# meyer-lab/cmtf-pls

Measured on AMD Instinct MI355X. Metric: nipals_iters_per_sec, higher is better.
Workload: dtype f32

## Files before the change

### cmtf_pls_amd/_lib.py

```python
from __future__ import annotations

import ctypes
import os
from ctypes import c_char_p, c_double, c_int, c_int64, c_size_t, c_uint64, c_void_p

_HERE = os.path.dirname(os.path.abspath(__file__))
LIB_PATH = os.environ.get("CMTFPLS_LIB") or os.path.join(_HERE, "lib", "libcmtfpls.so")

_P = c_void_p

class XcovBlock(ctypes.Structure):
    _fields_ = [("S", _P), ("S2", _P), ("colcnt", _P), ("n_samples", c_double), ("order", c_int), ("A", c_int), ("B", c_int),
                ("n_squarings", c_int), ("Z", _P), ("wA", _P), ("wB", _P), ("info", _P)]


class KfoldState(ctypes.Structure):
    _fields_ = [("I", c_int), ("A", c_int), ("B", c_int), ("M", c_int), ("K", c_int), ("R", c_int)] + [
        (name, _P) for name in ("fold_of", "S", "mean", "Yk", "Gy", "WA", "WB", "Q", "Wa", "Wb", "T", "Gt", "coef", "Rm", "tm",
                                "Tout", "vec", "n_iter", "status", "part")]


SIGNATURES = {
    "cmtfpls_xcov_iterate_blocks_f64": (c_int, [ctypes.POINTER(XcovBlock), c_int, c_int, _P, _P, _P, _P, _P, c_int, _P, c_size_t, _P]),
    "cmtfpls_abi_version": (c_int, []),
# ... 33 lines not shown
    "cmtfpls_project_rows2_f32": (c_int, [_P, c_int, c_int, _P, _P, _P, _P, c_int, c_int, _P, _P, _P, c_int64, c_int, _P, c_int, _P]),
    "cmtfpls_project_rows2_f64": (c_int, [_P, c_int, c_int, _P, _P, _P, _P, c_int, c_int, _P, _P, _P, c_int64, c_int, _P, c_int, _P]),
    "cmtfpls_project_rows_idx_f32": (c_int, [_P, _P, c_int64, c_int, c_int, c_int, _P, _P, _P, _P, c_int, _P]),
    "cmtfpls_project_rows_idx_f64": (c_int, [_P, _P, c_int64, c_int, c_int, c_int, _P, _P, _P, _P, c_int, _P]),
    "cmtfpls_project_rows2_idx_f32": (c_int, [_P, c_int, c_int, _P, _P, _P, _P, c_int, c_int, _P, _P, _P, _P, c_int64, c_int, _P, c_int, _P]),
    "cmtfpls_project_rows2_idx_f64": (c_int, [_P, c_int, c_int, _P, _P, _P, _P, c_int, c_int, _P, _P, _P, _P, c_int64, c_int, _P, c_int, _P]),
    "cmtfpls_allreduce_sum_f64": (c_int, [_P, _P, c_size_t, _P]),
    "cmtfpls_allreduce_sum_f32": (c_int, [_P, _P, c_size_t, _P]),
    "cmtfpls_axpy_scalar_f64": (c_int, [_P, c_int64, _P, _P, _P]),
    "cmtfpls_xcov_deflate_f32": (c_int, [_P, c_int64, c_int, c_int, _P, c_int, c_int, _P, _P, _P, _P, _P, _P, c_size_t, _P]),
    "cmtfpls_xcov_deflate_f64": (c_int, [_P, c_int64, c_int, c_int, _P, c_int, c_int, _P, _P, _P, _P, _P, _P, c_size_t, _P]),
    "cmtfpls_xcov_stats_workspace_bytes": (c_size_t, [c_int64, c_int64, c_int]),
    "cmtfpls_xcov_stats_f32": (c_int, [_P, c_int64, c_int64, _P, c_int, c_int, _P, _P, _P, c_size_t, _P]),
    "cmtfpls_xcov_stats_f64": (c_int, [_P, c_int64, c_int64, _P, c_int, c_int, _P, _P, _P, c_size_t, _P]),
    "cmtfpls_xcov_ssq_workspace_bytes": (c_size_t, [c_int64, c_int64, c_int]),
    "cmtfpls_xcov_ssq_f32": (c_int, [_P, c_int64, c_int64, _P, c_int, c_int, _P, _P, _P, _P, c_size_t, _P]),
    "cmtfpls_xcov_ssq_f64": (c_int, [_P, c_int64, c_int64, _P, c_int, c_int, _P, _P, _P, _P, c_size_t, _P]),
    "cmtfpls_score_contract_workspace_bytes": (c_size_t, [c_int64, c_int64]),
    "cmtfpls_score_contract_f32": (c_int, [_P, c_int64, c_int, c_int, _P, _P, _P, _P, _P, c_double, _P, _P, _P, _P, c_size_t, _P]),
    "cmtfpls_score_contract_f64": (c_int, [_P, c_int64, c_int, c_int, _P, _P, _P, _P, _P, c_double, _P, _P, _P, _P, c_size_t, _P]),
    "cmtfpls_kr_axpy_f64": (c_int, [_P, c_int, c_int, _P, _P, c_int, c_int, _P, _P]),
    "cmtfpls_xcov_f32_mixed": (c_int, [_P, c_int64, c_int64, _P, c_int, c_int, _P, c_int, _P, c_size_t, _P]),
    "cmtfpls_mttkrp_f32_mixed": (c_int, [_P, c_int64, c_int, c_int, _P, _P, c_int, _P, c_int, _P]),
    "cmtfpls_mttkrp_f32": (c_int, [_P, c_int64, c_int, c_int, _P, _P, c_int, _P, c_int, _P]),
    "cmtfpls_mttkrp_f64": (c_int, [_P, c_int64, c_int, c_int, _P, _P, c_int, _P, c_int, _P]),
    "cmtfpls_score_f32": (c_int, [_P, c_int64, c_int, c_int, _P, _P, _P, _P, _P]),
    "cmtfpls_score_f64": (c_int, [_P, c_int64, c_int, c_int, _P, _P, _P, _P, _P]),
    "cmtfpls_score_s_f64": (c_int, [_P, c_int, c_int, c_int, _P, _P, _P, _P]),
    "cmtfpls_deflate_contract_workspace_bytes": (c_size_t, [c_int64, c_int64]),
    "cmtfpls_deflate_contract_yq_f32": (c_int, [_P, c_int64, c_int, c_int, _P, _P, _P, _P, c_int, c_int, _P, _P, c_int, _P, _P, c_size_t, _P]),
    "cmtfpls_deflate_contract_yq_f64": (c_int, [_P, c_int64, c_int, c_int, _P, _P, _P, _P, c_int, c_int, _P, _P, c_int, _P, _P, c_size_t, _P]),
    "cmtfpls_score_gram_f32": (c_int, [_P, c_int64, c_int, c_int, _P, _P, _P, _P, _P, c_int, c_int, _P, _P]),
    "cmtfpls_score_gram_f64": (c_int, [_P, c_int64, c_int, c_int, _P, _P, _P, _P, _P, c_int, c_int, _P, _P]),
    "cmtfpls_q_update_f64": (c_int, [_P, c_int, c_int, _P, c_int, _P, _P, _P, _P]),
    "cmtfpls_deflate_f32": (c_int, [_P, c_int64, c_int, c_int, _P, _P, _P, _P, _P]),
    "cmtfpls_deflate_f64": (c_int, [_P, c_int64, c_int, c_int, _P, _P, _P, _P, _P]),
    "cmtfpls_score_deflate_f32": (c_int, [_P, c_int64, c_int, c_int, _P, _P, _P, _P, _P, _P]),
    "cmtfpls_score_deflate_f64": (c_int, [_P, c_int64, c_int, c_int, _P, _P, _P, _P, _P, _P]),
    "cmtfpls_small_workspace_bytes": (c_size_t, []),
    "cmtfpls_gram_tn_f64": (c_int, [_P, c_int, c_int, _P, c_int, c_int, c_int64, _P, _P, c_size_t, _P]),
    "cmtfpls_rowdot_f64": (c_int, [_P, c_int, c_int, c_int64, _P, _P, _P, _P, _P, c_size_t, _P]),
    "cmtfpls_scores_mean_f64": (c_int, [_P, c_int, c_int64, _P, _P]),
    "cmtfpls_y_deflate_f64": (c_int, [_P, c_int, c_int, c_int64, _P, c_int, c_int, _P, _P, _P, _P, c_size_t, _P]),
    "cmtfpls_sum_f64": (c_int, [_P, c_int64, _P, _P]),
    "cmtfpls_normal_solve_f64": (c_int, [_P, _P, c_int, _P, c_int, _P]),
    "cmtfpls_normal_solve_workspace_bytes": (c_size_t, [c_int]),
    "cmtfpls_normal_solve_ws_f64": (c_int, [_P, _P, c_int, _P, c_int, _P, c_size_t, _P]),
    "cmtfpls_unit_upper_solve_rows_f64": (c_int, [_P, c_int64, c_int, c_int, _P, _P, _P, _P]),
    "cmtfpls_kr_gram_row_f64": (c_int, [_P, c_int, c_int, c_int, _P, c_int, _P]),
    "cmtfpls_kr_gram_f64": (c_int, [_P, c_int, c_int, _P, c_int, c_double, _P]),
    "cmtfpls_khatri_rao_f64": (c_int, [_P, c_int, _P, c_int, c_int, _P, _P]),
    "cmtfpls_predict_rows_f64": (c_int, [_P, c_int64, c_int, c_int, _P, c_int, _P, _P, c_int, _P]),
    "cmtfpls_recon_f32": (c_int, [_P, c_int64, c_int, c_int, _P, _P, c_int, c_int, _P, _P, _P]),
    "cmtfpls_recon_f64": (c_int, [_P, c_int64, c_int, c_int, _P, _P, c_int, c_int, _P, _P, _P]),
    "cmtfpls_recon_r2_workspace_bytes": (c_size_t, [c_int64, c_int64]),
    "cmtfpls_recon_r2_f32": (c_int, [_P, _P, c_int64, c_int, c_int, _P, _P, c_int, c_int, _P, _P, _P, c_size_t, _P]),
    "cmtfpls_recon_r2_f64": (c_int, [_P, _P, c_int64, c_int, c_int, _P, _P, c_int, c_int, _P, _P, _P, c_size_t, _P]),
    "cmtfpls_resid_rows_workspace_bytes": (c_size_t, [c_int64, c_int64]),
    "cmtfpls_resid_rows_f32": (c_int, [_P, _P, c_int64, c_int, c_int, _P, _P, c_int, c_int, _P, _P, _P, _P, c_size_t, _P]),
    "cmtfpls_resid_rows_f64": (c_int, [_P, _P, c_int64, c_int, c_int, _P, _P, c_int, c_int, _P, _P, _P, _P, c_size_t, _P]),
    "cmtfpls_loo_fold_workspace_bytes": (c_size_t, [c_int, c_int, c_int, c_int, c_int]),
    "cmtfpls_loo_tpls_f64": (c_int, [_P, _P, _P, _P, c_int, c_int, c_int, c_int, c_int, c_double, c_int, c_int, c_int, _P, _P, _P, c_size_t, _P]),
    "cmtfpls_loo_xcov_fold_workspace_bytes": (c_size_t, [c_int, c_int, c_int, c_int, c_int]),
    "cmtfpls_kfold_xcov_workspace_bytes": (c_size_t, [c_int64, c_int64, c_int, c_int]),
    "cmtfpls_kfold_xcov_f32": (c_int, [_P, c_int64, c_int, c_int, _P, c_int, _P, _P, c_int, _P, _P, _P, _P, _P, c_size_t, _P]),
    "cmtfpls_kfold_xcov_f64": (c_int, [_P, c_int64, c_int, c_int, _P, c_int, _P, _P, c_int, _P, _P, _P, _P, _P, c_size_t, _P]),
# ... 59 lines not shown
```

### cmtf_pls_amd/backend.py

```python
from __future__ import annotations

import ctypes
from typing import Optional, Tuple

import torch

from . import _lib

_SUFFIX = {torch.float32: "f32", torch.float64: "f64"}


def _ptr(t: Optional[torch.Tensor]):
    return None if t is None else t.data_ptr()


class HipBackend:
    name = "hip"

    def __init__(self, device: Optional[torch.device] = None):
        self.lib = _lib.load()
        if not torch.cuda.is_available():
            raise _lib.CmtfplsError("cmtf_pls_amd needs a ROCm GPU (torch.cuda.is_available() is False); there is no CPU fallback")
        self.device = torch.device(device) if device is not None else torch.device("cuda", torch.cuda.current_device())
        self.n_partials = int(self.lib.cmtfpls_sweep_partials())
# ... 274 lines not shown
        assert WA.is_contiguous() and WB.is_contiguous() and out.stride(1) == 1
        fn = self.lib.cmtfpls_mttkrp_f32_mixed if (mixed and X2.dtype == torch.float32) else self._fn("mttkrp", X2)
        rc = fn(_ptr(X2), X2.shape[0], A, B, _ptr(WA), _ptr(WB), R, _ptr(out), out.stride(0), self._stream())
        if rc == 4:
            return None
        _lib.check(rc, "mttkrp")
        return out

    def score(self, X2, A, B, wA, wB, rowcnt, out) -> torch.Tensor:
        _lib.check(self._fn("score", X2)(_ptr(X2), X2.shape[0], A, B, _ptr(wA), _ptr(wB), _ptr(rowcnt), _ptr(out), self._stream()), "score")
        return out

    def score_s(self, S, A, B, wA, wB, out) -> torch.Tensor:
        assert S.dtype == torch.float64 and S.is_contiguous()
        _lib.check(self.lib.cmtfpls_score_s_f64(_ptr(S), S.shape[0], A, B, _ptr(wA), _ptr(wB), _ptr(out), self._stream()), "score_s")
        return out

    def score_contract(self, X2, A, B, wA, wB, shift, t, Z, sub_own=None, add_other=None, alpha: float = 1.0,
                       csum: Optional[torch.Tensor] = None) -> Optional[torch.Tensor]:
        I, P = X2.shape
        if not X2.is_contiguous() or P != A * B:
            return None
        for v in (sub_own, add_other):
            assert v is None or (v.is_contiguous() and v.numel() == I and v.dtype == torch.float64)
        nbytes = self.lib.cmtfpls_score_contract_workspace_bytes(I, P)
        ws = self._workspace("score_contract", max(nbytes, 256))
        rc = self._fn("score_contract", X2)(_ptr(X2), I, A, B, _ptr(wA), _ptr(wB), _ptr(shift), _ptr(sub_own), _ptr(add_other), float(alpha),
                                            _ptr(t), _ptr(Z), _ptr(csum), _ptr(ws), ws.numel(), self._stream())
        if rc == 4:
            return None
        _lib.check(rc, "score_contract")
        return Z

    def score_gram(self, X2, A, B, wA, wB, rowcnt, out, Y: torch.Tensor, qpart: torch.Tensor) -> Optional[torch.Tensor]:
        assert qpart.numel() >= self.n_partials * Y.shape[1] and qpart.is_contiguous()
        rc = self._fn("score_gram", X2)(_ptr(X2), X2.shape[0], A, B, _ptr(wA), _ptr(wB), _ptr(rowcnt), _ptr(out),
                                        _ptr(Y), Y.stride(0), Y.shape[1], _ptr(qpart), self._stream())
        if rc == 4:
            return None
        _lib.check(rc, "score_gram")
        return out

    def q_update(self, q: torch.Tensor, qpart: Optional[torch.Tensor] = None, normalize: bool = True,
                 G: Optional[torch.Tensor] = None, q_prev: Optional[torch.Tensor] = None,
                 du2: Optional[torch.Tensor] = None, nparts: Optional[int] = None) -> None:
        M = q.numel()
        nrows = (nparts or self.n_partials) if qpart is not None else 0
        assert qpart is None or (qpart.is_contiguous() and qpart.numel() >= nrows * M)
        _lib.check(self.lib.cmtfpls_q_update_f64(_ptr(qpart), nrows, M, _ptr(q), int(normalize),
                                                 _ptr(G), _ptr(q_prev), _ptr(du2), self._stream()), "q_update")

    def deflate(self, X2, A, B, t, wA, wB) -> torch.Tensor:
        part = self.empty(self.n_partials)
        _lib.check(self._fn("deflate", X2)(_ptr(X2), X2.shape[0], A, B, _ptr(t), _ptr(wA), _ptr(wB), _ptr(part), self._stream()), "deflate")
        return self._close_partials(part)

    def deflate_contract_yq(self, X2, A, B, t, wA, wB, Y: torch.Tensor, q: torch.Tensor, masked: bool,
                            out: torch.Tensor) -> Optional[torch.Tensor]:
        I, P = X2.shape
        ws = self._workspace("deflate_contract", self.lib.cmtfpls_deflate_contract_workspace_bytes(I, P))
        ssq = self.empty(1)
        rc = self._fn("deflate_contract_yq", X2)(_ptr(X2), I, A, B, _ptr(t), _ptr(wA), _ptr(wB), _ptr(Y), Y.stride(0), Y.shape[1],
                                                 _ptr(q), _ptr(out), int(masked), _ptr(ssq), _ptr(ws), ws.numel(), self._stream())
        if rc == 4:
            return None
        _lib.check(rc, "deflate_contract_yq")
        return ssq

    def score_deflate(self, X2, A, B, wA, wB, rowcnt, out) -> Optional[torch.Tensor]:
        part = self.empty(self.n_partials)
# ... 351 lines not shown
```

### cmtf_pls_amd/csrc/sweeps.hip

```cpp
#include "common.hpp"

namespace cmtfpls {

#ifndef CMTFPLS_CONTRACT_U
#define CMTFPLS_CONTRACT_U 4
#endif
constexpr int kContractU = CMTFPLS_CONTRACT_U;
constexpr int kYqChunk = 2048;
#ifndef CMTFPLS_YQ_UNFUSE_TILES
#define CMTFPLS_YQ_UNFUSE_TILES 16
#endif
constexpr int kYqUnfuseTiles = CMTFPLS_YQ_UNFUSE_TILES;

struct ContractPlan {
  int vec;
  int col_tiles;
  int row_blocks;
  int rows_per_block;
};

constexpr int kDcU = 2;

#ifndef CMTFPLS_CONTRACT_BLOCKS_FULL
#define CMTFPLS_CONTRACT_BLOCKS_FULL 512
// ... 610 lines not shown
      hipLaunchKernelGGL((deflate_contract_kernel<T, 0, false>), grid, dim3(kSweepThreads), 0, st, X, I, P, B, t, wA, wB, u_ws,
                         part, sspart, p.rows_per_block, nullptr, 0, 0, nullptr);
  } else if (masked)
    hipLaunchKernelGGL((deflate_contract_kernel<T, 1, true>), grid, dim3(kSweepThreads), lds, st, X, I, P, B, t, wA, wB, nullptr,
                       part, sspart, p.rows_per_block, Y, ldy, M, q);
  else
    hipLaunchKernelGGL((deflate_contract_kernel<T, 0, true>), grid, dim3(kSweepThreads), lds, st, X, I, P, B, t, wA, wB, nullptr,
                       part, sspart, p.rows_per_block, Y, ldy, M, q);
  launch_reduce_rows(part, p.row_blocks, P, Z, st);
  launch_reduce_rows(sspart, (int)nss, 1, ssq, st);
  return check_launch("deflate_contract_yq");
}

__device__ __forceinline__ void stage_loadings(double* sA, double* sB, const double* __restrict__ wA,
                                               const double* __restrict__ wB, int A, int B) {
  for (int i = threadIdx.x; i < A; i += blockDim.x) sA[i] = wA[i];
  for (int i = threadIdx.x; i < B; i += blockDim.x) sB[i] = wB[i];
  __syncthreads();
}
static inline size_t loadings_lds_bytes(int A, int B) { return ((size_t)((A + 1) & ~1) + (size_t)((B + 1) & ~1)) * sizeof(double); }

template <typename T, int V, bool MASKED>
__device__ __forceinline__ double dot_pack(const Pack<T, V>& x, const double* sBk) {
  double s = 0.0;
#pragma unroll
  for (int e = 0; e < V; ++e) {
    T xv = x.e[e];
    if (MASKED) xv = (xv == xv) ? xv : (T)0;
    s = fma((double)xv, sBk[e], s);
  }
  return s;
}

template <typename T, bool MASKED, bool VEC, bool GRAM, bool GL = false>
__global__ __launch_bounds__(kSweepThreads) __attribute__((amdgpu_waves_per_eu(5))) void score_kernel(
    const T* __restrict__ X, int64_t I, int A, int B, const double* __restrict__ wA,
    const double* __restrict__ wB, const double* __restrict__ rowcnt, double* __restrict__ t,
    const double* __restrict__ Y, int ldy, int M, double* __restrict__ qpart) {
  extern __shared__ double lds[];
  __shared__ double qs[kSweepThreads / kWave][kWave];
  double qacc = 0.0;
  const double* sA = GL ? wA : lds;
  const double* sB = GL ? wB : lds + ((A + 1) & ~1);
  if (!GL) stage_loadings(lds, lds + ((A + 1) & ~1), wA, wB, A, B);
  constexpr int V = VEC ? VecOf<T>::N : 1;
  using VT = Pack<T, V>;
  const int lane = threadIdx.x & 63;
  const int64_t P = (int64_t)A * B;
  const int64_t nwaves = (int64_t)gridDim.x * (kSweepThreads / kWave);
  const int64_t step = (int64_t)kWave * V;
  const int64_t c0 = (int64_t)lane * V;
  const KronWalk w0(c0, step, B);
  for (int64_t row = (int64_t)blockIdx.x * (kSweepThreads / kWave) + (threadIdx.x >> 6); row < I; row += nwaves) {
    const T* __restrict__ xr = X + row * P;
    double yv = 0.0;
    if (GRAM) yv = Y[row * ldy + ((lane < M) ? lane : 0)];
    double acc = 0.0;
    KronWalk w = w0;
    int64_t c = c0;
    constexpr int UN = kRowUnroll;
    for (; c + (UN - 1) * step < P; c += UN * step) {
      VT x[UN];
#pragma unroll
      for (int s = 0; s < UN; ++s) x[s] = ld_stream(reinterpret_cast<const VT*>(xr + c + s * step));
#pragma unroll
      for (int s = 0; s < UN; ++s) {
        acc = fma(sA[w.j], dot_pack<T, V, MASKED>(x[s], sB + w.k), acc);
        w.next();
      }
    }
    for (; c < P; c += step) {
      const VT x = ld_stream(reinterpret_cast<const VT*>(xr + c));
      acc = fma(sA[w.j], dot_pack<T, V, MASKED>(x, sB + w.k), acc);
      w.next();
    }
    acc = wave_sum(acc);
    const double ti = MASKED ? acc / rowcnt[row] * (double)P : acc;
    if (lane == 0) t[row] = ti;
    if (GRAM) qacc = fma(ti, yv, qacc);
  }
  if (GRAM) {
    qs[threadIdx.x >> 6][lane] = qacc;
    __syncthreads();
    if (threadIdx.x < M) {
      double tot = 0.0;
#pragma unroll
      for (int wv = 0; wv < kSweepThreads / kWave; ++wv) tot += qs[wv][threadIdx.x];
      qpart[(int64_t)blockIdx.x * M + threadIdx.x] = tot;
    }
  }
}

template <typename T, bool MASKED>
__global__ __launch_bounds__(1024) void score_fewrows_kernel(const T* __restrict__ X, int A, int B, const double* __restrict__ wA,
                                                            const double* __restrict__ wB, const double* __restrict__ rowcnt,
                                                            double* __restrict__ t) {
  extern __shared__ double lds[];
  __shared__ double red[16];
  const double* sA = lds;
  const double* sB = lds + ((A + 1) & ~1);
  stage_loadings(lds, lds + ((A + 1) & ~1), wA, wB, A, B);
  constexpr int V = VecOf<T>::N;
  using VT = Pack<T, V>;
  const int64_t P = (int64_t)A * B;
  const int64_t step = (int64_t)1024 * V;
  const int64_t row = blockIdx.x;
  const T* __restrict__ xr = X + row * P;
  KronWalk w((int64_t)threadIdx.x * V, step, B);
  double acc = 0.0;
  int64_t c = (int64_t)threadIdx.x * V;
  constexpr int UN = 4;
  for (; c + (UN - 1) * step < P; c += UN * step) {
    VT x[UN];
#pragma unroll
    for (int s = 0; s < UN; ++s) x[s] = ld_stream(reinterpret_cast<const VT*>(xr + c + s * step));
#pragma unroll
    for (int s = 0; s < UN; ++s) {
      acc = fma(sA[w.j], dot_pack<T, V, MASKED>(x[s], sB + w.k), acc);
      w.next();
    }
  }
// ... 367 lines not shown
template <typename T>
static int narrow_nvl(const T* X, int A, int B) {
#ifndef CMTFPLS_ROWS_NARROW
#define CMTFPLS_ROWS_NARROW 1
#endif
  constexpr int V = VecOf<T>::N;
  if (!CMTFPLS_ROWS_NARROW || (B % V) != 0 || (reinterpret_cast<uintptr_t>(X) & 15) != 0) return 0;
  const int64_t P = (int64_t)A * B;
  if (P <= 64 * V) return 1;
  if (P <= 2 * 64 * V) return 2;
  if (P <= 4 * 64 * V) return 4;
  return 0;
}

template <typename T, bool MASKED, bool GRAM, int OP>
static void launch_rows_narrow(int nvl, hipStream_t st, T* X, int64_t I, int A, int B, const double* wA, const double* wB,
                               const double* rowcnt, double* t, const double* Y, int ldy, int M, double* qpart, double* ssq_part) {
  const dim3 g(kSweepBlocks), b(kSweepThreads);
  if (nvl == 1) hipLaunchKernelGGL((rows_narrow_kernel<T, MASKED, GRAM, 1, OP>), g, b, 0, st, X, I, A, B, wA, wB, rowcnt, t, Y, ldy, M, qpart, ssq_part);
  else if (nvl == 2) hipLaunchKernelGGL((rows_narrow_kernel<T, MASKED, GRAM, 2, OP>), g, b, 0, st, X, I, A, B, wA, wB, rowcnt, t, Y, ldy, M, qpart, ssq_part);
  else hipLaunchKernelGGL((rows_narrow_kernel<T, MASKED, GRAM, 4, OP>), g, b, 0, st, X, I, A, B, wA, wB, rowcnt, t, Y, ldy, M, qpart, ssq_part);
}

template <typename T>
static bool vec_ok(const T* X, int B) {
  return (B % VecOf<T>::N == 0) && ((reinterpret_cast<uintptr_t>(X) & 15) == 0);
}
static bool shape_ok(int64_t I, int A, int B) { return I > 0 && A > 0 && B > 0; }
static constexpr size_t kMaxLoadingsLds = 96 * 1024;

template <typename T>
static int run_score(const T* X, int64_t I, int A, int B, const double* wA, const double* wB,
                     const double* rowcnt, double* t, hipStream_t st,
                     const double* Y = nullptr, int ldy = 0, int M = 0, double* qpart = nullptr, bool few_rows_ok = false) {
  if (!X || !wA || !wB || !t || !shape_ok(I, A, B)) { set_error("score: bad argument"); return CMTFPLS_EINVAL; }
  const bool gram = Y != nullptr;
  if (gram && (!qpart || M <= 0 || ldy < M)) { set_error("score_gram: bad argument"); return CMTFPLS_EINVAL; }
  if (gram && M > kWave) { set_error("score_gram: more than 64 responses; use score + gram_tn"); return CMTFPLS_EUNSUPPORTED; }
  if (const int nvl = narrow_nvl(X, A, B)) {
    T* Xm = const_cast<T*>(X);
    const bool msk = rowcnt != nullptr;
    if (gram) { if (msk) launch_rows_narrow<T, true, true, 0>(nvl, st, Xm, I, A, B, wA, wB, rowcnt, t, Y, ldy, M, qpart, nullptr);
                else launch_rows_narrow<T, false, true, 0>(nvl, st, Xm, I, A, B, wA, wB, rowcnt, t, Y, ldy, M, qpart, nullptr); }
    else      { if (msk) launch_rows_narrow<T, true, false, 0>(nvl, st, Xm, I, A, B, wA, wB, rowcnt, t, nullptr, 0, 0, nullptr, nullptr);
                else launch_rows_narrow<T, false, false, 0>(nvl, st, Xm, I, A, B, wA, wB, rowcnt, t, nullptr, 0, 0, nullptr, nullptr); }
    return check_launch("score");
  }
  size_t lds = loadings_lds_bytes(A, B);
  const bool gl = lds > kMaxLoadingsLds;
  if (gl) lds = 0;
  const bool v = vec_ok(X, B), m = rowcnt != nullptr;
  if (few_rows_ok && !gram && v && !gl && I <= 64 && (int64_t)A * B >= 8192) {
    if (m) hipLaunchKernelGGL((score_fewrows_kernel<T, true>), dim3((unsigned)I), dim3(1024), lds, st, X, A, B, wA, wB, rowcnt, t);
    else hipLaunchKernelGGL((score_fewrows_kernel<T, false>), dim3((unsigned)I), dim3(1024), lds, st, X, A, B, wA, wB, rowcnt, t);
    return check_launch("score");
  }
  const dim3 g(kSweepBlocks), b(kSweepThreads);
#define LAUNCH(MS, V, G) do { if (gl) hipLaunchKernelGGL((score_kernel<T, MS, V, G, true>), g, b, lds, st, X, I, A, B, wA, wB, rowcnt, t, Y, ldy, M, qpart); \
    else hipLaunchKernelGGL((score_kernel<T, MS, V, G, false>), g, b, lds, st, X, I, A, B, wA, wB, rowcnt, t, Y, ldy, M, qpart); } while (0)
  if (gram) { if (m && v) LAUNCH(true, true, true); else if (m) LAUNCH(true, false, true); else if (v) LAUNCH(false, true, true); else LAUNCH(false, false, true); }
  else      { if (m && v) LAUNCH(true, true, false); else if (m) LAUNCH(true, false, false); else if (v) LAUNCH(false, true, false); else LAUNCH(false, false, false); }
#undef LAUNCH
  return check_launch("score");
}

template <typename T>
static int run_deflate(T* X, int64_t I, int A, int B, const double* t, const double* wA, const double* wB,
                       double* ssq_part, hipStream_t st) {
  if (!X || !wA || !wB || !t || !shape_ok(I, A, B)) { set_error("deflate: bad argument"); return CMTFPLS_EINVAL; }
  if (const int nvl = narrow_nvl(X, A, B)) {
    launch_rows_narrow<T, false, false, 1>(nvl, st, X, I, A, B, wA, wB, nullptr, const_cast<double*>(t), nullptr, 0, 0, nullptr, ssq_part);
    return check_launch("deflate");
  }
  const size_t lds = loadings_lds_bytes(A, B);
  const dim3 g(kSweepBlocks), b(kSweepThreads);
  if (lds > kMaxLoadingsLds) {
    if (vec_ok(X, B)) hipLaunchKernelGGL((deflate_kernel<T, true, true>), g, b, 0, st, X, I, A, B, t, wA, wB, ssq_part);
    else hipLaunchKernelGGL((deflate_kernel<T, false, true>), g, b, 0, st, X, I, A, B, t, wA, wB, ssq_part);
    return check_launch("deflate");
  }
#ifndef CMTFPLS_DEFLATE_ROWS
#define CMTFPLS_DEFLATE_ROWS 1
#endif
  if (CMTFPLS_DEFLATE_ROWS && vec_ok(X, B)) {
    const int64_t P = (int64_t)A * B;
    constexpr int V = VecOf<T>::N;
    const bool kc = ((1024 * V) % B) == 0;
#ifndef CMTFPLS_DEFLATE_ROWS_PAD
#define CMTFPLS_DEFLATE_ROWS_PAD 81920
#endif
    const size_t lds_w = loadings_lds_bytes(A, B);
    const size_t lds = lds_w + ((lds_w + CMTFPLS_DEFLATE_ROWS_PAD + 1024 <= 160 * 1024) ? CMTFPLS_DEFLATE_ROWS_PAD : 0);
    if (P > (int64_t)256 * V * 4 && P <= (int64_t)1024 * V * 4) {
      if (kc) hipLaunchKernelGGL((deflate_rows_kernel<T, 4, 1024, true>), g, dim3(1024), lds, st, X, I, A, B, t, wA, wB, ssq_part);
// ... 120 lines not shown
    else launch_rows_narrow<T, false, false, 2>(nvl, st, X, I, A, B, wA, wB, rowcnt, t, nullptr, 0, 0, nullptr, ssq_part);
    return check_launch("score_deflate");
  }
  const size_t lds = loadings_lds_bytes(A, B);
  if (lds > kMaxLoadingsLds) { set_error("score_deflate: loadings exceed LDS"); return CMTFPLS_EUNSUPPORTED; }
  const bool v = vec_ok(X, B), m = rowcnt != nullptr;
  const int V = v ? VecOf<T>::N : 1;
  const int64_t P = (int64_t)A * B;
  int threads = 256, nv = 1;
  if (P > (int64_t)256 * V * 4) { threads = 1024; nv = 4; }
  if (P > (int64_t)1024 * V * 16) { set_error("score_deflate: row does not fit one workgroup; use score + deflate"); return CMTFPLS_EUNSUPPORTED; }
  while ((int64_t)threads * V * nv < P) nv *= 4;
  if (threads == 1024 && nv == 16 && lds + (size_t)1024 * 8 * 16 + 1024 > (size_t)160 * 1024) {
    set_error("score_deflate: loadings + the parked half row exceed the LDS; use score + deflate");
    return CMTFPLS_EUNSUPPORTED;
  }
  const bool kc = v && ((threads * V) % B == 0);
  const bool full = kc && ((int64_t)threads * V * nv == P);
  if (m && full) launch_sd<T, true, true, 2>(nv, threads, lds, st, X, I, A, B, wA, wB, rowcnt, t, ssq_part);
  else if (m && kc) launch_sd<T, true, true, 1>(nv, threads, lds, st, X, I, A, B, wA, wB, rowcnt, t, ssq_part);
  else if (m && v) launch_sd<T, true, true, 0>(nv, threads, lds, st, X, I, A, B, wA, wB, rowcnt, t, ssq_part);
  else if (m) launch_sd<T, true, false, 0>(nv, threads, lds, st, X, I, A, B, wA, wB, rowcnt, t, ssq_part);
  else if (full) launch_sd<T, false, true, 2>(nv, threads, lds, st, X, I, A, B, wA, wB, rowcnt, t, ssq_part);
  else if (kc) launch_sd<T, false, true, 1>(nv, threads, lds, st, X, I, A, B, wA, wB, rowcnt, t, ssq_part);
  else if (v) launch_sd<T, false, true, 0>(nv, threads, lds, st, X, I, A, B, wA, wB, rowcnt, t, ssq_part);
  else launch_sd<T, false, false, 0>(nv, threads, lds, st, X, I, A, B, wA, wB, rowcnt, t, ssq_part);
  return check_launch("score_deflate");
}

}

using namespace cmtfpls;

extern "C" {

int cmtfpls_sweep_partials(void) { return kSweepBlocks; }

size_t cmtfpls_mode0_contract_workspace_bytes(int64_t I, int64_t P) {
  if (I <= 0 || P <= 0) return 0;
  int rb = 1;
  for (int elem = 4; elem <= 8; elem += 4)
    for (int U = 2; U <= kContractU; U += 2)
      for (int which = 0; which < 2; ++which) {
        const int r = plan_contract(I, P, elem, U, which ? kContractBlocks : kContractBlocksFull).row_blocks;
        if (r > rb) rb = r;
      }
  return (size_t)rb * (size_t)P * sizeof(double) + (size_t)I * sizeof(double);
}
size_t cmtfpls_colstats_workspace_bytes(int64_t I, int64_t P) { return 2 * cmtfpls_mode0_contract_workspace_bytes(I, P); }

int cmtfpls_colstats_f32(const float* X, int64_t I, int64_t P, double* colsum, double* colcnt, void* ws, size_t n, void* s) {
  return run_contract<float, 2>(X, I, P, nullptr, colsum, colcnt, ws, n, (hipStream_t)s);
}
int cmtfpls_colstats_f64(const double* X, int64_t I, int64_t P, double* colsum, double* colcnt, void* ws, size_t n, void* s) {
  return run_contract<double, 2>(X, I, P, nullptr, colsum, colcnt, ws, n, (hipStream_t)s);
}
int cmtfpls_mode0_contract_f32(const float* X, int64_t I, int64_t P, const double* u, double* Z, int masked, void* ws, size_t n, void* s) {
  return masked ? run_contract<float, 1>(X, I, P, u, Z, nullptr, ws, n, (hipStream_t)s)
                : run_contract<float, 0>(X, I, P, u, Z, nullptr, ws, n, (hipStream_t)s);
}
int cmtfpls_mode0_contract_f64(const double* X, int64_t I, int64_t P, const double* u, double* Z, int masked, void* ws, size_t n, void* s) {
  return masked ? run_contract<double, 1>(X, I, P, u, Z, nullptr, ws, n, (hipStream_t)s)
                : run_contract<double, 0>(X, I, P, u, Z, nullptr, ws, n, (hipStream_t)s);
}
int cmtfpls_mode0_contract_yq_f32(const float* X, int64_t I, int64_t P, const double* Y, int ldy, int M, const double* q,
                                  double* Z, int masked, void* ws, size_t n, void* s) {
// ... 3 lines not shown
int cmtfpls_mode0_contract_yq_f64(const double* X, int64_t I, int64_t P, const double* Y, int ldy, int M, const double* q,
                                  double* Z, int masked, void* ws, size_t n, void* s) {
  return masked ? run_contract<double, 1>(X, I, P, nullptr, Z, nullptr, ws, n, (hipStream_t)s, Y, ldy, M, q)
                : run_contract<double, 0>(X, I, P, nullptr, Z, nullptr, ws, n, (hipStream_t)s, Y, ldy, M, q);
}
size_t cmtfpls_deflate_contract_workspace_bytes(int64_t I, int64_t P) {
  if (I <= 0 || P <= 0) return 0;
  const ContractPlan a = plan_contract(I, P, 4, kDcU), b = plan_contract(I, P, 8, kDcU);
  const size_t na = (size_t)a.row_blocks * ((size_t)P + a.col_tiles), nb = (size_t)b.row_blocks * ((size_t)P + b.col_tiles);
  const size_t colform = ((na > nb ? na : nb) + (size_t)I) * sizeof(double);
  const size_t rowform = ((size_t)kDcRowsGrid * (size_t)P + (size_t)kDcRowsGrid + (size_t)I) * sizeof(double);
  return colform > rowform ? colform : rowform;
}
int cmtfpls_deflate_contract_yq_f32(float* X, int64_t I, int A, int B, const double* t, const double* wA, const double* wB,
                                    const double* Y, int ldy, int M, const double* q, double* Z, int masked, double* ssq,
                                    void* ws, size_t n, void* s) {
  return run_deflate_contract<float>(X, I, A, B, t, wA, wB, Y, ldy, M, q, Z, masked, ssq, ws, n, (hipStream_t)s);
}
int cmtfpls_deflate_contract_yq_f64(double* X, int64_t I, int A, int B, const double* t, const double* wA, const double* wB,
                                    const double* Y, int ldy, int M, const double* q, double* Z, int masked, double* ssq,
                                    void* ws, size_t n, void* s) {
  return run_deflate_contract<double>(X, I, A, B, t, wA, wB, Y, ldy, M, q, Z, masked, ssq, ws, n, (hipStream_t)s);
}
int cmtfpls_score_gram_f32(const float* X, int64_t I, int A, int B, const double* wA, const double* wB, const double* rowcnt,
                           double* t, const double* Y, int ldy, int M, double* qpart, void* s) {
  if (!Y) { set_error("score_gram: Y is null"); return CMTFPLS_EINVAL; }
  return run_score<float>(X, I, A, B, wA, wB, rowcnt, t, (hipStream_t)s, Y, ldy, M, qpart);
}
int cmtfpls_score_gram_f64(const double* X, int64_t I, int A, int B, const double* wA, const double* wB, const double* rowcnt,
                           double* t, const double* Y, int ldy, int M, double* qpart, void* s) {
  if (!Y) { set_error("score_gram: Y is null"); return CMTFPLS_EINVAL; }
  return run_score<double>(X, I, A, B, wA, wB, rowcnt, t, (hipStream_t)s, Y, ldy, M, qpart);
}
int cmtfpls_center_f32(float* X, int64_t I, int64_t P, const double* mean, double* rowcnt, double* ssq_part, void* s) {
  return run_center<float>(X, I, P, mean, rowcnt, ssq_part, (hipStream_t)s);
}
int cmtfpls_center_f64(double* X, int64_t I, int64_t P, const double* mean, double* rowcnt, double* ssq_part, void* s) {
  return run_center<double>(X, I, P, mean, rowcnt, ssq_part, (hipStream_t)s);
}
int cmtfpls_score_f32(const float* X, int64_t I, int A, int B, const double* wA, const double* wB, const double* rowcnt, double* t, void* s) {
  return run_score<float>(X, I, A, B, wA, wB, rowcnt, t, (hipStream_t)s);
}
int cmtfpls_score_s_f64(const double* S, int M, int A, int B, const double* wA, const double* wB, double* tq, void* s) {
  return run_score<double>(S, M, A, B, wA, wB, nullptr, tq, (hipStream_t)s, nullptr, 0, 0, nullptr, true);
}
int cmtfpls_score_f64(const double* X, int64_t I, int A, int B, const double* wA, const double* wB, const double* rowcnt, double* t, void* s) {
  return run_score<double>(X, I, A, B, wA, wB, rowcnt, t, (hipStream_t)s);
}
int cmtfpls_deflate_f32(float* X, int64_t I, int A, int B, const double* t, const double* wA, const double* wB, double* ssq_part, void* s) {
  return run_deflate<float>(X, I, A, B, t, wA, wB, ssq_part, (hipStream_t)s);
}
int cmtfpls_deflate_f64(double* X, int64_t I, int A, int B, const double* t, const double* wA, const double* wB, double* ssq_part, void* s) {
  return run_deflate<double>(X, I, A, B, t, wA, wB, ssq_part, (hipStream_t)s);
}
int cmtfpls_score_deflate_f32(float* X, int64_t I, int A, int B, const double* wA, const double* wB, const double* rowcnt, double* t, double* ssq_part, void* s) {
  return run_score_deflate<float>(X, I, A, B, wA, wB, rowcnt, t, ssq_part, (hipStream_t)s);
}
int cmtfpls_score_deflate_f64(double* X, int64_t I, int A, int B, const double* wA, const double* wB, const double* rowcnt, double* t, double* ssq_part, void* s) {
  return run_score_deflate<double>(X, I, A, B, wA, wB, rowcnt, t, ssq_part, (hipStream_t)s);
}

}
```

### cmtf_pls_amd/fitrun.py

```python
from __future__ import annotations

import math
from typing import Dict, List, Optional

import numpy as np
import torch

from .fitrun_xcov import XcovMixin
from .state import BlockState, FitState, split_trailing, validate_limits


class FitRun(XcovMixin):

    def __init__(self, eng: NipalsEngine, Xs: List[torch.Tensor], Y: torch.Tensor, n_components: int, coupled: bool,
                 algorithm: str = "direct", owned: Optional[List[bool]] = None, allow_raw: bool = True):
        be, comm = eng.be, eng.comm
        Xs = list(Xs)
        owned = [True] * len(Xs) if owned is None else list(owned)
        if algorithm not in ("direct", "xcov"):
            raise ValueError("algorithm must be 'direct' or 'xcov'")
        self.algorithm_requested = self.algorithm = algorithm
        self.notes: List[str] = []
        validate_limits([tuple(X.shape) for X in Xs], n_components)
        self.eng, self.Xs, self.Y, self.R, self.coupled = eng, Xs, Y, n_components, coupled
# ... 66 lines not shown
        self.Zs = [be.empty(blk.A * blk.B) for blk in self.blocks]
        self.fac = [be.zeros(len(blk.shape) - 1, max(blk.shape[1:])) if len(blk.shape) > 3 else None for blk in self.blocks]
        self.tol = 1e-8
        self.Ts = be.empty(len(self.blocks), I)
        self.t = self.Ts[0] if (len(self.blocks) == 1 and not coupled) else be.empty(I)
        self.status = be.zeros(1 + 2 * len(self.blocks))
        self.status[1::2] = 1.0
        self.status_host = None
        if self.status.is_cuda:
            self.status_host = torch.empty(self.status.shape, dtype=torch.float64, pin_memory=True)
        self.sq_max = int(getattr(be, "rank1_squarings", 30))
        self.sq_budget = [self.sq_max] * len(self.blocks)
        side = int(getattr(be, "rank1_chain_side", 0))
        self.sq_spare = [3 if (len(blk.shape) == 3 and min(blk.A, blk.B) <= side) else 1 for blk in self.blocks]
        self.u = be.empty(I)
        self.u_new = be.empty(I)
        self.q = be.empty(M)
        self.n_iter: List[int] = []
        self.pipeline_stats = {"iterations": 0, "ahead": 0, "unused": 0, "waited": 0, "redone": 0}
        self._executed = 0
        self._parity = 0
        self.mixed = False
        self.use_graphs = False
        self._graphs = {}
        self._graph_error = None
        self._collectives_captured = None
        self._z_ready = False
        self._fused = (algorithm == "direct" and M <= 64
                       and all(hasattr(be, f) for f in ("mode0_contract_yq", "score_gram", "q_update")))
        if self._fused:
            self.Gy = be.empty(M, M)
            self.qbuf = [be.zeros(M), be.zeros(M)]
            self.qpart = be.empty(len(self.blocks), int(be.n_partials) * M)
        elif algorithm == "direct" and comm.sharded:
            self.Gy = be.empty(M, M)
            self.q_prev = be.zeros(M)
        if algorithm == "xcov":
            nb = len(self.blocks)
            self._s_pair = 2 * M <= 64 and eng.opt.xcov_pair_build
            self.S, self.S2, self.S12 = [], [], []
            for blk in self.blocks:
                if blk.has_miss and self._s_pair:
                    both = be.empty(2 * M, blk.A * blk.B)
                    self.S12.append(both)
                    self.S.append(both[:M])
                    self.S2.append(both[M:])
                else:
                    self.S12.append(None)
                    pre = self._s_prebuilt.get(len(self.S))
                    self.S.append(pre if pre is not None else be.empty(M, blk.A * blk.B))
                    self.S2.append(be.empty(M, blk.A * blk.B) if blk.has_miss else None)
            self.rowscale = [(float(blk.A * blk.B) / blk.rowcnt) if blk.has_miss else None for blk in self.blocks]
            any_miss = any(blk.has_miss for blk in self.blocks)
            self.Yw = be.empty(I, 2 * M if self._s_pair else M) if any_miss else None
            self.Gy = be.empty(M, M)
            self.Tq = be.empty(nb, M)
            self.qx = [be.zeros(M), be.zeros(M)]
            self.qc = self.qx[0]
            self.qn = self.Tq[0] if (nb == 1 and not coupled) else be.empty(M)
            self._s_carry = (not any(blk.has_miss for blk in self.blocks)
                             and all(hasattr(be, f) for f in ("s_downdate", "deflate_contract_yq")))
            self._s_ready = False
            self._nowrite = False
            if self.raw:
                self.zM = be.zeros(M)
                self.zA = [be.zeros(blk.A) for blk in self.blocks]
# ... 252 lines not shown
                    seg_colscale()
                self._run(("loadings", budgets), seg_loadings_scores)
                comm.allreduce(self.q)
                self._run(("yupdate", it > 0, par), seg_y_update)
            host = self._read_status()
            local, peer = self._update_budgets(host), self._peer_failed(host, first)
            if not (local or peer):
                break
            first = False
        if sharded:
            self.q_prev.copy_(self.q)
        self._parity ^= 1
        return None if it == 0 else math.sqrt(max(float(host[0]), 0.0))

    def _iterate_fused(self, it: int) -> Optional[float]:
        be, comm = self.eng.be, self.eng.comm
        self._executed += 1
        sharded = comm.sharded
        par = self._parity
        q_cur, q_new = self.qbuf[par], self.qbuf[par ^ 1]
        nparts = len(self.blocks) * int(be.n_partials)

        def seg_contract():
            for b, blk in enumerate(self.blocks):
                if be.mode0_contract_yq(self.X2[b], self.Y, q_cur, blk.has_miss, out=self.Zs[b]) is None:
                    be.rowdot(self.Y, q_cur, self.u, None)
                    be.mode0_contract(self.X2[b], self.u, blk.has_miss, out=self.Zs[b])

        def seg_colscale():
            for b, blk in enumerate(self.blocks):
                if blk.has_miss:
                    be.colscale(self.Zs[b], blk.colcnt, self.n_total)

        def seg_loadings_scores():
            for b, blk in enumerate(self.blocks):
                self.eng._rank1(blk, self.Zs[b], self.wA[b], self.wB[b], info=self.status[1 + 2 * b: 3 + 2 * b],
                                n_squarings=self.sq_budget[b], fac=self.fac[b], tol=self.tol)
                if be.score_gram(self.X2[b], blk.A, blk.B, self.wA[b], self.wB[b], blk.rowcnt if blk.has_miss else None,
                                 self.Ts[b], self.Y, self.qpart[b]) is None:
                    raise RuntimeError("score_gram refused a shape the fused iteration was planned for")
            if sharded:
                be.q_update(q_new, self.qpart, normalize=False, nparts=nparts)

        def seg_y_update():
            if sharded:
                be.q_update(q_new, None, normalize=True, G=self.Gy, q_prev=q_cur, du2=self.status[0:1])
            else:
                be.q_update(q_new, self.qpart, normalize=True, G=self.Gy, q_prev=q_cur, du2=self.status[0:1], nparts=nparts)

        have_z = self._z_ready and it == 0
        self._z_ready = False
        first = True
        while True:
            budgets = tuple(self.sq_budget)
            if not sharded:
                def whole():
                    if first:
                        if not have_z:
                            seg_contract()
                        seg_colscale()
                    seg_loadings_scores()
                    seg_y_update()
                self._run(("fiter", par, budgets, first, have_z), whole)
            else:
                def whole_sharded():
                    if first:
                        if not have_z:
                            seg_contract()
                        for b in range(len(self.blocks)):
                            comm.allreduce(self.Zs[b])
                        seg_colscale()
                    seg_loadings_scores()
                    comm.allreduce(q_new)
                    seg_y_update()
                if not self._run_with_collectives(("fiter+ar", par, budgets, first, have_z), whole_sharded):
                    if first:
                        if not have_z:
                            self._run(("fcontract", par), seg_contract)
                        for b in range(len(self.blocks)):
                            comm.allreduce(self.Zs[b])
# ... 230 lines not shown
```

### include/cmtfpls.h

```cpp
#ifndef CMTFPLS_H
#define CMTFPLS_H

#include <stddef.h>
#include <stdint.h>

#ifdef __cplusplus
extern "C" {
#endif

#define CMTFPLS_OK 0
#define CMTFPLS_EINVAL 1
#define CMTFPLS_EWORKSPACE 2
#define CMTFPLS_EHIP 3
#define CMTFPLS_EUNSUPPORTED 4

int cmtfpls_abi_version(void);
const char* cmtfpls_last_error(void);
int cmtfpls_clear_error(void);
int cmtfpls_status_to_host(const void* src, void* dst_host, size_t bytes, void* event, void* stream);

size_t cmtfpls_colstats_workspace_bytes(int64_t I, int64_t P);
int cmtfpls_colstats_f32(const float* X, int64_t I, int64_t P, double* colsum, double* colcnt,
                         void* ws, size_t ws_bytes, void* stream);
int cmtfpls_colstats_f64(const double* X, int64_t I, int64_t P, double* colsum, double* colcnt,
// ... 79 lines not shown
                               void* ws, size_t ws_bytes, void* stream);
int cmtfpls_score_contract_f64(const double* X, int64_t I, int A, int B, const double* wA, const double* wB, const double* shift,
                               const double* sub_own, const double* add_other, double alpha, double* t, double* Z, double* csum,
                               void* ws, size_t ws_bytes, void* stream);
int cmtfpls_xcov_f32_mixed(const float* X, int64_t I, int64_t P, const double* Y, int ldy, int M, double* S,
                           int masked, void* ws, size_t ws_bytes, void* stream);
int cmtfpls_mttkrp_f32_mixed(const float* X, int64_t I, int A, int B, const double* WA, const double* WB, int R,
                             double* out, int ldo, void* stream);

int cmtfpls_mttkrp_f32(const float* X, int64_t I, int A, int B, const double* WA, const double* WB, int R,
                       double* out, int ldo, void* stream);
int cmtfpls_mttkrp_f64(const double* X, int64_t I, int A, int B, const double* WA, const double* WB, int R,
                       double* out, int ldo, void* stream);

int cmtfpls_score_f32(const float* X, int64_t I, int A, int B, const double* wA, const double* wB,
                      const double* rowcnt, double* t, void* stream);
int cmtfpls_score_f64(const double* X, int64_t I, int A, int B, const double* wA, const double* wB,
                      const double* rowcnt, double* t, void* stream);
int cmtfpls_score_s_f64(const double* S, int M, int A, int B, const double* wA, const double* wB, double* tq, void* stream);

size_t cmtfpls_deflate_contract_workspace_bytes(int64_t I, int64_t P);
int cmtfpls_deflate_contract_yq_f32(float* X, int64_t I, int A, int B, const double* t, const double* wA,
                                    const double* wB, const double* Y, int ldy, int M, const double* q, double* Z,
                                    int masked, double* ssq, void* ws, size_t ws_bytes, void* stream);
int cmtfpls_deflate_contract_yq_f64(double* X, int64_t I, int A, int B, const double* t, const double* wA,
                                    const double* wB, const double* Y, int ldy, int M, const double* q, double* Z,
                                    int masked, double* ssq, void* ws, size_t ws_bytes, void* stream);
int cmtfpls_score_gram_f32(const float* X, int64_t I, int A, int B, const double* wA, const double* wB,
                           const double* rowcnt, double* t, const double* Y, int ldy, int M, double* qpart,
                           void* stream);
int cmtfpls_score_gram_f64(const double* X, int64_t I, int A, int B, const double* wA, const double* wB,
                           const double* rowcnt, double* t, const double* Y, int ldy, int M, double* qpart,
                           void* stream);
int cmtfpls_q_update_f64(const double* qpart, int nblk, int M, double* q, int normalize, const double* G,
                         const double* q_prev, double* du2, void* stream);

int cmtfpls_deflate_f32(float* X, int64_t I, int A, int B, const double* t, const double* wA,
                        const double* wB, double* ssq_part, void* stream);
int cmtfpls_deflate_f64(double* X, int64_t I, int A, int B, const double* t, const double* wA,
                        const double* wB, double* ssq_part, void* stream);

int cmtfpls_score_deflate_f32(float* X, int64_t I, int A, int B, const double* wA, const double* wB,
                              const double* rowcnt, double* t, double* ssq_part, void* stream);
int cmtfpls_score_deflate_f64(double* X, int64_t I, int A, int B, const double* wA, const double* wB,
                              const double* rowcnt, double* t, double* ssq_part, void* stream);

size_t cmtfpls_small_workspace_bytes(void);
int cmtfpls_gram_tn_f64(const double* A, int lda, int a, const double* B, int ldb, int b, int64_t I,
                        double* C, void* ws, size_t ws_bytes, void* stream);
int cmtfpls_rowdot_f64(const double* Y, int ldy, int M, int64_t I, const double* q, double* u,
                       const double* u_old, double* du2, void* ws, size_t ws_bytes, void* stream);
int cmtfpls_scores_mean_f64(const double* Ts, int nb, int64_t I, double* out, void* stream);
int cmtfpls_y_deflate_f64(double* Y, int ldy, int M, int64_t I, const double* T, int ldt, int R,
                          const double* b, const double* q, double* ssq, void* ws, size_t ws_bytes,
                          void* stream);
int cmtfpls_sum_f64(const double* in, int64_t n, double* out, void* stream);

int cmtfpls_project_rows_f32(const float* X, int64_t I, int A, int B, int R, const double* WA, const double* WB,
                             const double* mean, double* scores, int ld, void* stream);
int cmtfpls_project_rows_f64(const double* X, int64_t I, int A, int B, int R, const double* WA, const double* WB,
                             const double* mean, double* scores, int ld, void* stream);
int cmtfpls_project_rows2_f32(const float* X0, int A0, int B0, const double* WA0, const double* WB0, const double* mean0,
                              const float* X1, int A1, int B1, const double* WA1, const double* WB1, const double* mean1,
                              int64_t I, int R, double* scores, int ld, void* stream);
int cmtfpls_project_rows2_f64(const double* X0, int A0, int B0, const double* WA0, const double* WB0, const double* mean0,
                              const double* X1, int A1, int B1, const double* WA1, const double* WB1, const double* mean1,
// ... 126 lines not shown
```

Before: 768.7.

## Fold q update into score_gram kernel via last-block reduction

Adds a score_gram_q kernel variant in which the last block to finish, found with an atomic counter, reduces the per-block q partials, normalises q and computes du2 inside the score kernel. The fit loop uses it for single-block, unsharded runs and then skips the separate q_update launch. This removes one kernel launch and its dependency gap per NIPALS iteration. In exchange it adds atomics, relaxed agent-scope stores and a serial tail on one block. The qcount buffer comes from be.zeros(1), whose dtype is not unsigned, which may be a subtle mismatch.

Measured after the change: 768.2 (median of 4 runs). Within noise of the previous version (-0.1%).

```diff
diff --git a/cmtf_pls_amd/_lib.py b/cmtf_pls_amd/_lib.py
--- a/cmtf_pls_amd/_lib.py
+++ b/cmtf_pls_amd/_lib.py
@@ -89,6 +89,8 @@
     "cmtfpls_deflate_contract_yq_f64": (c_int, [_P, c_int64, c_int, c_int, _P, _P, _P, _P, c_int, c_int, _P, _P, c_int, _P, _P, c_size_t, _P]),
     "cmtfpls_score_gram_f32": (c_int, [_P, c_int64, c_int, c_int, _P, _P, _P, _P, _P, c_int, c_int, _P, _P]),
     "cmtfpls_score_gram_f64": (c_int, [_P, c_int64, c_int, c_int, _P, _P, _P, _P, _P, c_int, c_int, _P, _P]),
+    "cmtfpls_score_gram_q_f32": (c_int, [_P, c_int64, c_int, c_int, _P, _P, _P, _P, _P, c_int, c_int, _P, _P, _P, _P, _P, _P, _P]),
+    "cmtfpls_score_gram_q_f64": (c_int, [_P, c_int64, c_int, c_int, _P, _P, _P, _P, _P, c_int, c_int, _P, _P, _P, _P, _P, _P, _P]),
     "cmtfpls_q_update_f64": (c_int, [_P, c_int, c_int, _P, c_int, _P, _P, _P, _P]),
     "cmtfpls_deflate_f32": (c_int, [_P, c_int64, c_int, c_int, _P, _P, _P, _P, _P]),
     "cmtfpls_deflate_f64": (c_int, [_P, c_int64, c_int, c_int, _P, _P, _P, _P, _P]),
diff --git a/cmtf_pls_amd/backend.py b/cmtf_pls_amd/backend.py
--- a/cmtf_pls_amd/backend.py
+++ b/cmtf_pls_amd/backend.py
@@ -330,10 +330,19 @@
         _lib.check(rc, "score_contract")
         return Z
 
-    def score_gram(self, X2, A, B, wA, wB, rowcnt, out, Y: torch.Tensor, qpart: torch.Tensor) -> Optional[torch.Tensor]:
+    score_folds_y_update = True
+
+    def score_gram(self, X2, A, B, wA, wB, rowcnt, out, Y: torch.Tensor, qpart: torch.Tensor,
+                   y_update: Optional[tuple] = None) -> Optional[torch.Tensor]:
         assert qpart.numel() >= self.n_partials * Y.shape[1] and qpart.is_contiguous()
-        rc = self._fn("score_gram", X2)(_ptr(X2), X2.shape[0], A, B, _ptr(wA), _ptr(wB), _ptr(rowcnt), _ptr(out),
-                                        _ptr(Y), Y.stride(0), Y.shape[1], _ptr(qpart), self._stream())
+        if y_update is not None:
+            count, q, G, q_prev, du2 = y_update
+            rc = self._fn("score_gram_q", X2)(_ptr(X2), X2.shape[0], A, B, _ptr(wA), _ptr(wB), _ptr(rowcnt), _ptr(out),
+                                              _ptr(Y), Y.stride(0), Y.shape[1], _ptr(qpart), _ptr(count), _ptr(q), _ptr(G),
+                                              _ptr(q_prev), _ptr(du2), self._stream())
+        else:
+            rc = self._fn("score_gram", X2)(_ptr(X2), X2.shape[0], A, B, _ptr(wA), _ptr(wB), _ptr(rowcnt), _ptr(out),
+                                            _ptr(Y), Y.stride(0), Y.shape[1], _ptr(qpart), self._stream())
         if rc == 4:
             return None
         _lib.check(rc, "score_gram")
diff --git a/cmtf_pls_amd/csrc/sweeps.hip b/cmtf_pls_amd/csrc/sweeps.hip
--- a/cmtf_pls_amd/csrc/sweeps.hip
+++ b/cmtf_pls_amd/csrc/sweeps.hip
@@ -666,11 +666,94 @@
   return s;
 }
 
-template <typename T, bool MASKED, bool VEC, bool GRAM, bool GL = false>
+struct QFinish {
+  unsigned* count;
+  double* q;
+  const double* G;
+  const double* q_prev;
+  double* du2;
+};
+
+__device__ __forceinline__ double sc1_ld(const double* p) {
+  return __longlong_as_double((long long)__hip_atomic_load(reinterpret_cast<const unsigned long long*>(p), __ATOMIC_RELAXED, __HIP_MEMORY_SCOPE_AGENT));
+}
+__device__ __forceinline__ void sc1_st(double* p, double v) {
+  __hip_atomic_store(reinterpret_cast<unsigned long long*>(p), (unsigned long long)__double_as_longlong(v), __ATOMIC_RELAXED, __HIP_MEMORY_SCOPE_AGENT);
+}
+
+__device__ __forceinline__ void q_finish_last(const double* qpart, int nblk, int M, const QFinish& f) {
+  __shared__ double part[64 * 17];
+  __shared__ double qs[64];
+  __shared__ double dq[64];
+  __shared__ double red[16];
+  const int tid = threadIdx.x, lane = tid & 63, wv = tid >> 6;
+  const int Mp = (M <= 16) ? 16 : (M <= 32) ? 32 : 64;
+  const int ngrp = 1024 / Mp, gstep = kSweepThreads / Mp;
+  const int m = tid & (Mp - 1), g0 = tid / Mp;
+  const int msafe = (m < M) ? m : 0;
+  double sacc[4] = {0.0, 0.0, 0.0, 0.0};
+  const int nj = (nblk + ngrp - 1) / ngrp;
+  for (int j0 = 0; j0 < nj; j0 += 4) {
+    double v[4][4];
+#pragma unroll
+    for (int r = 0; r < 4; ++r)
+#pragma unroll
+      for (int jj = 0; jj < 4; ++jj) {
+        const int b = g0 + r * gstep + (j0 + jj) * ngrp;
+        v[r][jj] = sc1_ld(qpart + (int64_t)((b < nblk) ? b : nblk - 1) * M + msafe);
+      }
+#pragma unroll
+    for (int r = 0; r < 4; ++r)
+#pragma unroll
+      for (int jj = 0; jj < 4; ++jj)
+        if (g0 + r * gstep + (j0 + jj) * ngrp < nblk) sacc[r] += v[r][jj];
+  }
+#pragma unroll
+  for (int r = 0; r < 4; ++r) part[(g0 + r * gstep) * (Mp + 1) + m] = (m < M) ? sacc[r] : 0.0;
+  __syncthreads();
+  if (tid < M) {
+    double tot = 0.0;
+    for (int g = 0; g < ngrp; ++g) tot += part[g * (Mp + 1) + tid];
+    qs[tid] = tot;
+  }
+  __syncthreads();
+  if (tid < 64) {
+    double v = (lane < M) ? qs[lane] : 0.0;
+    const double nrm = sqrt(wave_sum(v * v));
+    v = v / nrm;
+    if (lane < M) {
+      f.q[lane] = v;
+      dq[lane] = v - f.q_prev[lane];
+    }
+  }
+  __syncthreads();
+  double ws[4];
+#pragma unroll
+  for (int r = 0; r < 4; ++r) {
+    double sacc2 = 0.0;
+    for (int idx = tid + kSweepThreads * r; idx < M * M; idx += 1024) {
+      const int i = idx / M, j = idx - i * M;
+      sacc2 = fma(dq[i] * f.G[idx], dq[j], sacc2);
+    }
+    ws[r] = wave_sum(sacc2);
+  }
+  if (lane == 0) {
+#pragma unroll
+    for (int r = 0; r < 4; ++r) red[wv + 4 * r] = ws[r];
+  }
+  __syncthreads();
+  if (tid == 0) {
+    double s = 0.0;
+    for (int w = 0; w < 16; ++w) s += red[w];
+    f.du2[0] = s;
+  }
+}
+
+template <typename T, bool MASKED, bool VEC, bool GRAM, bool GL = false, bool QF = false>
 __global__ __launch_bounds__(kSweepThreads) __attribute__((amdgpu_waves_per_eu(5))) void score_kernel(
     const T* __restrict__ X, int64_t I, int A, int B, const double* __restrict__ wA,
     const double* __restrict__ wB, const double* __restrict__ rowcnt, double* __restrict__ t,
-    const double* __restrict__ Y, int ldy, int M, double* __restrict__ qpart) {
+    const double* __restrict__ Y, int ldy, int M, double* __restrict__ qpart, QFinish qf) {
   extern __shared__ double lds[];
   __shared__ double qs[kSweepThreads / kWave][kWave];
   double qacc = 0.0;
@@ -720,7 +803,21 @@
       double tot = 0.0;
 #pragma unroll
       for (int wv = 0; wv < kSweepThreads / kWave; ++wv) tot += qs[wv][threadIdx.x];
-      qpart[(int64_t)blockIdx.x * M + threadIdx.x] = tot;
+      if (QF) sc1_st(qpart + (int64_t)blockIdx.x * M + threadIdx.x, tot);
+      else qpart[(int64_t)blockIdx.x * M + threadIdx.x] = tot;
+    }
+    if (QF) {
+      __shared__ int s_last;
+      if (threadIdx.x < kWave) {
+        asm volatile("s_waitcnt vmcnt(0)" ::: "memory");
+        if (threadIdx.x == 0)
+          s_last = __hip_atomic_fetch_add(qf.count, 1u, __ATOMIC_RELAXED, __HIP_MEMORY_SCOPE_AGENT) == gridDim.x - 1;
+      }
+      __syncthreads();
+      if (s_last) {
+        if (threadIdx.x == 0) __hip_atomic_store(qf.count, 0u, __ATOMIC_RELAXED, __HIP_MEMORY_SCOPE_AGENT);
+        q_finish_last(qpart, (int)gridDim.x, M, qf);
+      }
     }
   }
 }
@@ -1154,11 +1251,13 @@
 template <typename T>
 static int run_score(const T* X, int64_t I, int A, int B, const double* wA, const double* wB,
                      const double* rowcnt, double* t, hipStream_t st,
-                     const double* Y = nullptr, int ldy = 0, int M = 0, double* qpart = nullptr, bool few_rows_ok = false) {
+                     const double* Y = nullptr, int ldy = 0, int M = 0, double* qpart = nullptr, bool few_rows_ok = false,
+                     const QFinish* qf = nullptr) {
   if (!X || !wA || !wB || !t || !shape_ok(I, A, B)) { set_error("score: bad argument"); return CMTFPLS_EINVAL; }
   const bool gram = Y != nullptr;
   if (gram && (!qpart || M <= 0 || ldy < M)) { set_error("score_gram: bad argument"); return CMTFPLS_EINVAL; }
   if (gram && M > kWave) { set_error("score_gram: more than 64 responses; use score + gram_tn"); return CMTFPLS_EUNSUPPORTED; }
+  if (qf && narrow_nvl(X, A, B)) { set_error("score_gram_q: short rows; use score_gram + q_update"); return CMTFPLS_EUNSUPPORTED; }
   if (const int nvl = narrow_nvl(X, A, B)) {
     T* Xm = const_cast<T*>(X);
     const bool msk = rowcnt != nullptr;
@@ -1178,10 +1277,13 @@
     return check_launch("score");
   }
   const dim3 g(kSweepBlocks), b(kSweepThreads);
-#define LAUNCH(MS, V, G) do { if (gl) hipLaunchKernelGGL((score_kernel<T, MS, V, G, true>), g, b, lds, st, X, I, A, B, wA, wB, rowcnt, t, Y, ldy, M, qpart); \
-    else hipLaunchKernelGGL((score_kernel<T, MS, V, G, false>), g, b, lds, st, X, I, A, B, wA, wB, rowcnt, t, Y, ldy, M, qpart); } while (0)
-  if (gram) { if (m && v) LAUNCH(true, true, true); else if (m) LAUNCH(true, false, true); else if (v) LAUNCH(false, true, true); else LAUNCH(false, false, true); }
-  else      { if (m && v) LAUNCH(true, true, false); else if (m) LAUNCH(true, false, false); else if (v) LAUNCH(false, true, false); else LAUNCH(false, false, false); }
+  const QFinish q0{};
+#define LAUNCH(MS, V, G, F) do { \
+    if (gl) hipLaunchKernelGGL((score_kernel<T, MS, V, G, true, F>), g, b, lds, st, X, I, A, B, wA, wB, rowcnt, t, Y, ldy, M, qpart, F ? *qf : q0); \
+    else hipLaunchKernelGGL((score_kernel<T, MS, V, G, false, F>), g, b, lds, st, X, I, A, B, wA, wB, rowcnt, t, Y, ldy, M, qpart, F ? *qf : q0); } while (0)
+  if (gram && qf) { if (m && v) LAUNCH(true, true, true, true); else if (m) LAUNCH(true, false, true, true); else if (v) LAUNCH(false, true, true, true); else LAUNCH(false, false, true, true); }
+  else if (gram) { if (m && v) LAUNCH(true, true, true, false); else if (m) LAUNCH(true, false, true, false); else if (v) LAUNCH(false, true, true, false); else LAUNCH(false, false, true, false); }
+  else { if (m && v) LAUNCH(true, true, false, false); else if (m) LAUNCH(true, false, false, false); else if (v) LAUNCH(false, true, false, false); else LAUNCH(false, false, false, false); }
 #undef LAUNCH
   return check_launch("score");
 }
@@ -1368,6 +1470,15 @@
 
 using namespace cmtfpls;
 
+template <typename T>
+static int run_score_gram_q(const T* X, int64_t I, int A, int B, const double* wA, const double* wB, const double* rowcnt, double* t,
+                            const double* Y, int ldy, int M, double* qpart, unsigned* count, double* q, const double* G,
+                            const double* q_prev, double* du2, hipStream_t st) {
+  if (!Y || !count || !q || !G || !q_prev || !du2) { set_error("score_gram_q: bad argument"); return CMTFPLS_EINVAL; }
+  const QFinish qf{count, q, G, q_prev, du2};
+  return run_score<T>(X, I, A, B, wA, wB, rowcnt, t, st, Y, ldy, M, qpart, false, &qf);
+}
+
 extern "C" {
 
 int cmtfpls_sweep_partials(void) { return kSweepBlocks; }
@@ -1437,6 +1548,16 @@
   if (!Y) { set_error("score_gram: Y is null"); return CMTFPLS_EINVAL; }
   return run_score<double>(X, I, A, B, wA, wB, rowcnt, t, (hipStream_t)s, Y, ldy, M, qpart);
 }
+int cmtfpls_score_gram_q_f32(const float* X, int64_t I, int A, int B, const double* wA, const double* wB, const double* rowcnt,
+                             double* t, const double* Y, int ldy, int M, double* qpart, unsigned* count, double* q,
+                             const double* G, const double* q_prev, double* du2, void* s) {
+  return run_score_gram_q<float>(X, I, A, B, wA, wB, rowcnt, t, Y, ldy, M, qpart, count, q, G, q_prev, du2, (hipStream_t)s);
+}
+int cmtfpls_score_gram_q_f64(const double* X, int64_t I, int A, int B, const double* wA, const double* wB, const double* rowcnt,
+                             double* t, const double* Y, int ldy, int M, double* qpart, unsigned* count, double* q,
+                             const double* G, const double* q_prev, double* du2, void* s) {
+  return run_score_gram_q<double>(X, I, A, B, wA, wB, rowcnt, t, Y, ldy, M, qpart, count, q, G, q_prev, du2, (hipStream_t)s);
+}
 int cmtfpls_center_f32(float* X, int64_t I, int64_t P, const double* mean, double* rowcnt, double* ssq_part, void* s) {
   return run_center<float>(X, I, P, mean, rowcnt, ssq_part, (hipStream_t)s);
 }
diff --git a/cmtf_pls_amd/fitrun.py b/cmtf_pls_amd/fitrun.py
--- a/cmtf_pls_amd/fitrun.py
+++ b/cmtf_pls_amd/fitrun.py
@@ -122,6 +122,8 @@
             self.Gy = be.empty(M, M)
             self.qbuf = [be.zeros(M), be.zeros(M)]
             self.qpart = be.empty(len(self.blocks), int(be.n_partials) * M)
+            self._fold_q = not comm.sharded and len(self.blocks) == 1 and getattr(be, "score_folds_y_update", False)
+            self.qcount = be.zeros(1) if self._fold_q else None
         elif algorithm == "direct" and comm.sharded:
             self.Gy = be.empty(M, M)
             self.q_prev = be.zeros(M)
@@ -440,11 +442,18 @@
                 if blk.has_miss:
                     be.colscale(self.Zs[b], blk.colcnt, self.n_total)
 
+        q_folded = []
+
         def seg_loadings_scores():
+            q_folded.clear()
             for b, blk in enumerate(self.blocks):
                 self.eng._rank1(blk, self.Zs[b], self.wA[b], self.wB[b], info=self.status[1 + 2 * b: 3 + 2 * b],
                                 n_squarings=self.sq_budget[b], fac=self.fac[b], tol=self.tol)
-                if be.score_gram(self.X2[b], blk.A, blk.B, self.wA[b], self.wB[b], blk.rowcnt if blk.has_miss else None,
+                if self._fold_q and be.score_gram(self.X2[b], blk.A, blk.B, self.wA[b], self.wB[b],
+                                                  blk.rowcnt if blk.has_miss else None, self.Ts[b], self.Y, self.qpart[b],
+                                                  y_update=(self.qcount, q_new, self.Gy, q_cur, self.status[0:1])) is not None:
+                    q_folded.append(True)
+                elif be.score_gram(self.X2[b], blk.A, blk.B, self.wA[b], self.wB[b], blk.rowcnt if blk.has_miss else None,
                                  self.Ts[b], self.Y, self.qpart[b]) is None:
                     raise RuntimeError("score_gram refused a shape the fused iteration was planned for")
             if sharded:
@@ -453,7 +462,7 @@
         def seg_y_update():
             if sharded:
                 be.q_update(q_new, None, normalize=True, G=self.Gy, q_prev=q_cur, du2=self.status[0:1])
-            else:
+            elif not q_folded:
                 be.q_update(q_new, self.qpart, normalize=True, G=self.Gy, q_prev=q_cur, du2=self.status[0:1], nparts=nparts)
 
         have_z = self._z_ready and it == 0
diff --git a/include/cmtfpls.h b/include/cmtfpls.h
--- a/include/cmtfpls.h
+++ b/include/cmtfpls.h
@@ -135,6 +135,12 @@
 int cmtfpls_score_gram_f64(const double* X, int64_t I, int A, int B, const double* wA, const double* wB,
                            const double* rowcnt, double* t, const double* Y, int ldy, int M, double* qpart,
                            void* stream);
+int cmtfpls_score_gram_q_f32(const float* X, int64_t I, int A, int B, const double* wA, const double* wB,
+                             const double* rowcnt, double* t, const double* Y, int ldy, int M, double* qpart,
+                             unsigned* count, double* q, const double* G, const double* q_prev, double* du2, void* stream);
+int cmtfpls_score_gram_q_f64(const double* X, int64_t I, int A, int B, const double* wA, const double* wB,
+                             const double* rowcnt, double* t, const double* Y, int ldy, int M, double* qpart,
+                             unsigned* count, double* q, const double* G, const double* q_prev, double* du2, void* stream);
 int cmtfpls_q_update_f64(const double* qpart, int nblk, int M, double* q, int normalize, const double* G,
                          const double* q_prev, double* du2, void* stream);
 
```
